# jedeschaud/ct_icp

Measured on NVIDIA B200. Metric: scans/sec (RegisterFrame) on 64-beam ~120k-pt clouds, higher is better.
Workload: dtype f64

## Files before the change

ct_icp_b200/csrc/device_map.cu:

```cuda
#include "device_map.h"

#include <cooperative_groups.h>
#include "gather.cuh"
#include "frame_policy.h"

#include <algorithm>
#include <cstdio>
#include <cstdlib>
#include <numeric>
#include <stdexcept>
#include <vector>

namespace cticp {

#define CT_CUDA_CHECK(expr)                                                                              \
    do {                                                                                                 \
        cudaError_t _e = (expr);                                                                         \
        if (_e != cudaSuccess)                                                                           \
            throw CudaError(std::string(#expr) + ": " + cudaGetErrorString(_e) + " @" + __FILE__ + ":" + \
                            std::to_string(__LINE__));                                                   \
    } while (0)

__global__ void k_clear_level(MapLevel L) {
    const uint32_t cap = L.cap_mask + 1;
// ... 25 lines not shown
                k = atomicCAS(&L.slots[h].key, kEmptyKey, key);
                if (k == kEmptyKey) {
                    atomicAdd(&ctr->num_voxels, 1u);
                    slot = (int) h;
                    break;
                }
            }
            if (k == key) {
                slot = (int) h;
                break;
            }
            h = (h + 1) & L.cap_mask;
        }
        if (slot < 0) {
            atomicExch(&ctr->overflow, 1u);
            next[i] = kNil;
            continue;
        }
        const int old = atomicExch(&L.head[slot], i);
        next[i] = old;
        if (old == kNil) touched[atomicAdd(&ctr->num_touched, 1u)] = (uint32_t) slot;
    }
}
__global__ void k_insert_claim(MapLevel L, MapCounters *ctr, const double *__restrict__ world, const int *d_n,
                               int *__restrict__ next, uint32_t *__restrict__ touched) {
    insert_claim_dev(L, ctr, world, *d_n, next, touched);
}

constexpr int kInsertWarps = 4;
constexpr int kMaxCand = 512;
// ... 45 lines not shown
                    const int v = s_cand[w][a];
                    int rank = 0;
                    for (int b = 0; b < n; ++b) rank += (s_cand[w][b] < v);
                    s_sorted[w][rank] = v;
                }
                m = n;
            } else {
                int best = 0x7fffffff;
                for (int c = L.head[slot]; c != kNil; c = next[c])
                    if (c > last && c < best) best = c;
                if (lane == 0) s_sorted[w][0] = best;
                last = best;
                m = 1;
            }
            __syncwarp();
            for (int a = 0; a < m && count < L.B; ++a) {
                const int c = s_sorted[w][a];
                const double lx = world[3 * c] - ox, ly = world[3 * c + 1] - oy, lz = world[3 * c + 2] - oz;
                bool too_close = false;
                for (int j = lane; j < count; j += 32) {
                    const float4 q = s_pts[w][j];
                    const double dx = (double) q.x - lx, dy = (double) q.y - ly, dz = (double) q.z - lz;
                    const double d2 = dx * dx + dy * dy + dz * dz;
                    too_close |= !(d2 > L.min_dist2);
                }
                const bool reject = __any_sync(0xffffffffu, too_close);
                if (!reject) {
                    if (lane == 0) {
                        const float4 v = make_float4((float) lx, (float) ly, (float) lz, (float) (frame_ordinal + 1));
                        s_pts[w][count] = v;
                        gpts[count] = v;
                    }
                    ++count;
                }
                __syncwarp();
            }
            processed += m;
        }
        if (lane == 0) {
            L.slots[slot].count = (uint32_t) count;
            L.head[slot] = kNil;
            if (count > count0) atomicAdd(&ctr->num_points, (unsigned long long) (count - count0));
        }
        __syncwarp();
        if (L.normals && count > count0 && count >= 5) {
            double sx = 0, sy = 0, sz = 0, sxx = 0, sxy = 0, sxz = 0, syy = 0, syz = 0, szz = 0;
            for (int j = lane; j < count; j += 32) {
                const float4 q = s_pts[w][j];
                const double x = (double) q.x, y = (double) q.y, z = (double) q.z;
                sx += x; sy += y; sz += z;
// ... 66 lines not shown
    const int *d_n;
    double *world;
    Q4 qb, qe;
    V3 tb, te;
    SlerpConsts sc;
    V3 location;
    double max_distance;
    int do_remove, do_insert;
    int *next;
    uint32_t *touched;
    const double *frame_origins;
    int frame_ordinal;
    const FrameVerdict *verdict;
    double *frame_origins_mut;
};
__global__ void __launch_bounds__(kInsertWarps * 32)
k_map_update_fused(FusedUpdateArgs a) {
    namespace cg = cooperative_groups;
    cg::grid_group grid = cg::this_grid();
    __shared__ CommitScratch sc;
    if (a.verdict) {
        const FrameVerdict &v = *a.verdict;
        const int action = v.action;
        if (action != kFrameEvict && action != kFrameInsert) return;
        a.qb = Q4{v.state.qb[0], v.state.qb[1], v.state.qb[2], v.state.qb[3]};
        a.qe = Q4{v.state.qe[0], v.state.qe[1], v.state.qe[2], v.state.qe[3]};
        a.tb = V3{v.state.tb[0], v.state.tb[1], v.state.tb[2]};
        a.te = V3{v.state.te[0], v.state.te[1], v.state.te[2]};
        a.sc = v.sc;
        a.location = a.te;
        a.do_insert = action == kFrameInsert;
// ... 400 lines not shown
```

ct_icp_b200/csrc/engine.cu:

```cuda
#include "engine.h"

#include <algorithm>
#include <atomic>
#include <chrono>
#include <cmath>
#include <cstdio>
#include <cstdlib>
#include <cstring>

#include <emmintrin.h>
#include <xmmintrin.h>

#include <nvtx3/nvToolsExt.h>

namespace cticp {

#define CT_CUDA_CHECK(expr)                                                                              \
    do {                                                                                                 \
        cudaError_t _e = (expr);                                                                         \
        if (_e != cudaSuccess)                                                                           \
            throw CudaError(std::string(#expr) + ": " + cudaGetErrorString(_e) + " @" + __FILE__ + ":" + \
                            std::to_string(__LINE__));                                                   \
    } while (0)

// ... 663 lines not shown
    const bool needs_lo = PackScan(scan, sc.t_min, sc.t_max, pipe_->Staging());
    float4 *stage_lo = needs_lo ? pipe_->StagingLo() : nullptr;
    if (needs_lo) PackLoPlane(scan, sc.t_min, sc.t_max, stage_lo);
    CT_CUDA_CHECK(cudaMalloc(&sc.d_points, sizeof(float4) * n));
    CT_CUDA_CHECK(cudaMemcpyAsync(sc.d_points, pipe_->Staging(), sizeof(float4) * n, cudaMemcpyHostToDevice, stream_));
    if (needs_lo) {
        CT_CUDA_CHECK(cudaMalloc(&sc.d_lo, sizeof(float4) * n));
        CT_CUDA_CHECK(cudaMemcpyAsync(sc.d_lo, stage_lo, sizeof(float4) * n, cudaMemcpyHostToDevice, stream_));
    }
    CT_CUDA_CHECK(cudaStreamSynchronize(stream_));
    staged_.push_back(sc);
    return (int64_t) staged_.size() - 1;
}
void Engine::ClearStaged() {
    CT_CUDA_CHECK(cudaSetDevice(device_));
    CT_CUDA_CHECK(cudaStreamSynchronize(stream_));
    for (auto &sc : staged_) { cudaFree(sc.d_points); cudaFree(sc.d_lo); }
    staged_.clear();
}
void Engine::TimerStart() {
    CT_CUDA_CHECK(cudaSetDevice(device_));
    CT_CUDA_CHECK(cudaEventRecord(timer_ev_[0], stream_));
}
double Engine::TimerStop() {
    CT_CUDA_CHECK(cudaSetDevice(device_));
    CT_CUDA_CHECK(cudaEventRecord(timer_ev_[1], stream_));
    CT_CUDA_CHECK(cudaEventSynchronize(timer_ev_[1]));
    float ms = 0.f;
    CT_CUDA_CHECK(cudaEventElapsedTime(&ms, timer_ev_[0], timer_ev_[1]));
    return (double) ms;
// ... 757 lines not shown
```

ct_icp_b200/csrc/frame_pipeline.cu:

```cuda
#include "frame_pipeline.h"

#include <cooperative_groups.h>
#include <cstdlib>

#include <algorithm>
#include <cstring>

namespace cticp {

#define CT_CUDA_CHECK(expr)                                                                              \
    do {                                                                                                 \
        cudaError_t _e = (expr);                                                                         \
        if (_e != cudaSuccess)                                                                           \
            throw CudaError(std::string(#expr) + ": " + cudaGetErrorString(_e) + " @" + __FILE__ + ":" + \
                            std::to_string(__LINE__));                                                   \
    } while (0)

constexpr unsigned long long kGridEmpty = ~0ull;
constexpr size_t kMaxTiles = 4096;
constexpr int kTileShift = 10, kTile = 1 << kTileShift, kTileThreads = kTile / 4;

__device__ __forceinline__ unsigned long long short_voxel_key(const RawPoint &p, double voxel_size) {
    const double inv = 1.0 / voxel_size;
    const short x = (short) voxel_coord_rcp(p.x, voxel_size, inv);
    const short y = (short) voxel_coord_rcp(p.y, voxel_size, inv);
    const short z = (short) voxel_coord_rcp(p.z, voxel_size, inv);
    return ((unsigned long long) (unsigned short) x << 32) | ((unsigned long long) (unsigned short) y << 16) |
           (unsigned long long) (unsigned short) z;
}

__device__ __forceinline__ void grid_claim_dev(const float4 *pts, const float4 *lo, int n, double voxel_size, int use_perm,
                                               uint64_t seed, uint64_t counter, unsigned long long *keys,
                                               unsigned long long *vals, uint32_t cap_mask, int *__restrict__ slot_of) {
    const Perm perm = perm_make(seed, counter, (uint32_t) max(n, 1));
    for (int i = blockIdx.x * blockDim.x + threadIdx.x; i < n; i += gridDim.x * blockDim.x) {
        const unsigned long long key = short_voxel_key(load_raw(pts, lo, i), voxel_size);
        const uint32_t prio = use_perm ? perm_apply(perm, (uint32_t) i) : (uint32_t) i;
        uint32_t h = hash_key(key) & cap_mask;
        while (true) {
            unsigned long long k = *reinterpret_cast<volatile unsigned long long *>(&keys[h]);
            if (k == kGridEmpty) k = atomicCAS(&keys[h], kGridEmpty, key);
            if (k == kGridEmpty || k == key) break;
            h = (h + 1) & cap_mask;
        }
        atomicMin(&vals[h], ((unsigned long long) prio << 32) | (unsigned) i);
        slot_of[i] = (int) h;
    }
}
__global__ void k_grid_claim(const float4 *__restrict__ pts, const float4 *__restrict__ lo, const int *__restrict__ d_n,
                             double voxel_size, int use_perm, uint64_t seed, uint64_t counter, unsigned long long *keys,
                             unsigned long long *vals, uint32_t cap_mask, int *__restrict__ slot_of) {
    grid_claim_dev(pts, lo, *d_n, voxel_size, use_perm, seed, counter, keys, vals, cap_mask, slot_of);
}
__device__ __forceinline__ void grid_mark_dev(int n, int use_perm, uint64_t seed, uint64_t counter,
                                              const unsigned long long *vals, const int *slot_of, uint32_t *__restrict__ flags,
                                              uint32_t *__restrict__ src, uint32_t *__restrict__ tile_count) {
    const Perm perm = perm_make(seed, counter, (uint32_t) max(n, 1));
    for (int i = blockIdx.x * blockDim.x + threadIdx.x; i < n; i += gridDim.x * blockDim.x) {
        const uint32_t prio = use_perm ? perm_apply(perm, (uint32_t) i) : (uint32_t) i;
        const unsigned long long mine = ((unsigned long long) prio << 32) | (unsigned) i;
        if (vals[slot_of[i]] == mine) {
            flags[prio] = 1u;
            src[prio] = (uint32_t) i;
            atomicAdd(&tile_count[prio >> kTileShift], 1u);
        }
    }
}
__global__ void k_grid_mark(const int *__restrict__ d_n, int use_perm, uint64_t seed, uint64_t counter,
                            const unsigned long long *__restrict__ vals, const int *__restrict__ slot_of,
                            uint32_t *__restrict__ flags, uint32_t *__restrict__ src,
                            uint32_t *__restrict__ tile_count) {
    grid_mark_dev(*d_n, use_perm, seed, counter, vals, slot_of, flags, src, tile_count);
}
struct EmitScratch {
    uint32_t red[2][kTileThreads / 32];
    uint32_t warp[kTileThreads / 32];
    uint32_t before, total;
};
__device__ __forceinline__ uint32_t grid_emit_dev(const float4 *pts, const float4 *lo, const uint32_t *in_src_index, int n,
                                                  const uint32_t *flags, const uint32_t *src, const uint32_t *tile_count,
                                                  int use_perm2, uint64_t seed, uint64_t counter2, int override_alpha,
                                                  float alpha_value, float4 *__restrict__ out, float4 *__restrict__ out_lo,
                                                  uint32_t *__restrict__ out_src_index, int *__restrict__ d_total,
                                                  EmitScratch &sc) {
    uint32_t (&s_red)[2][kTileThreads / 32] = sc.red;
    uint32_t (&s_warp)[kTileThreads / 32] = sc.warp;
    uint32_t &s_before = sc.before, &s_total = sc.total;
    const int num_tiles = (n + kTile - 1) >> kTileShift;
    const int tid = threadIdx.x, lane = tid & 31, w = tid >> 5;
    uint32_t tot = 0;
    for (int t = tid; t < num_tiles; t += kTileThreads) tot += tile_count[t];
#pragma unroll
    for (int o = 16; o > 0; o >>= 1) tot += __shfl_xor_sync(0xffffffffu, tot, o);
    if (lane == 0) s_red[1][w] = tot;
    __syncthreads();
    if (tid == 0) {
        uint32_t b = 0;
        for (int i = 0; i < kTileThreads / 32; ++i) b += s_red[1][i];
        s_total = b;
    }
    __syncthreads();
    const uint32_t total = s_total;
    if (blockIdx.x == 0 && tid == 0) *d_total = (int) total;
    const Perm perm2 = perm_make(seed, counter2, max(total, 1u));

    for (int tile = blockIdx.x; tile < num_tiles; tile += gridDim.x) {
        uint32_t before = 0;
        for (int t = tid; t < tile; t += kTileThreads) before += tile_count[t];
#pragma unroll
        for (int o = 16; o > 0; o >>= 1) before += __shfl_xor_sync(0xffffffffu, before, o);
        __syncthreads();
        if (lane == 0) s_red[0][w] = before;
        const int p0 = (tile << kTileShift) + tid * 4;
        uint32_t v[4];
#pragma unroll
        for (int k = 0; k < 4; ++k) v[k] = (p0 + k < n) ? flags[p0 + k] : 0u;
        const uint32_t tsum = v[0] + v[1] + v[2] + v[3];
        uint32_t incl = tsum;
#pragma unroll
// ... 12 lines not shown
                const uint32_t c = s_warp[i];
                s_warp[i] = run;
                run += c;
            }
        }
        __syncthreads();
        uint32_t excl = s_before + s_warp[w] + (incl - tsum);
#pragma unroll
        for (int k = 0; k < 4; ++k) {
            if (v[k]) {
                const uint32_t dst = (use_perm2 && total > 1) ? perm_apply(perm2, excl) : excl;
                const uint32_t i = src[p0 + k];
                float4 val = pts[i];
                if (override_alpha) val.w = alpha_value;
                out[dst] = val;
                if (out_lo) {
                    float4 l = lo ? lo[i] : make_float4(0.f, 0.f, 0.f, 0.f);
                    if (override_alpha) l.w = 0.f;
                    out_lo[dst] = l;
                }
                out_src_index[dst] = in_src_index ? in_src_index[i] : i;
            }
            excl += v[k];
        }
    }
    return total;
}
__global__ void __launch_bounds__(kTileThreads)
k_grid_emit(const float4 *__restrict__ pts, const float4 *__restrict__ lo, const uint32_t *__restrict__ in_src_index,
            const int *__restrict__ d_n, const uint32_t *__restrict__ flags, const uint32_t *__restrict__ src,
            const uint32_t *__restrict__ tile_count, int use_perm2, uint64_t seed, uint64_t counter2,
            int override_alpha, float alpha_value, float4 *__restrict__ out, float4 *__restrict__ out_lo,
            uint32_t *__restrict__ out_src_index, int *__restrict__ d_total) {
    __shared__ EmitScratch sc;
    grid_emit_dev(pts, lo, in_src_index, *d_n, flags, src, tile_count, use_perm2, seed, counter2, override_alpha, alpha_value,
                  out, out_lo, out_src_index, d_total, sc);
}

struct FusedSampleArgs {
    const float4 *raw;
    const float4 *raw_lo;
    float4 *frame_lo, *kp_lo;
    int *counts;
    double voxel1, voxel2;
    uint64_t seed, c1, c2;
    int override_alpha;
    float alpha_value;
    unsigned long long *grid;
    uint32_t cap1;
    int *slot_of;
    uint32_t *tile1, *flags1, *src1;
    uint32_t *tile2, *flags2, *src2;
    float4 *frame, *keypoints;
    uint32_t *frame_src, *kp_src;
    int pre_cleared;
    uint32_t clear_words;
};
__global__ void __launch_bounds__(kTileThreads)
k_sample_fused(FusedSampleArgs a) {
    namespace cg = cooperative_groups;
    cg::grid_group grid = cg::this_grid();
    __shared__ EmitScratch sc;
    const size_t gtid = (size_t) blockIdx.x * blockDim.x + threadIdx.x, gsize = (size_t) gridDim.x * blockDim.x;
    const int n = a.counts[0];
    if (!a.pre_cleared) {
        for (size_t i = gtid; i < 2 * (size_t) a.cap1; i += gsize) a.grid[i] = kGridEmpty;
        for (size_t i = gtid; i < kMaxTiles + (size_t) n; i += gsize) a.tile1[i] = 0u;
        grid.sync();
    }
    grid_claim_dev(a.raw, a.raw_lo, n, a.voxel1, 1, a.seed, a.c1, a.grid, a.grid + a.cap1, a.cap1 - 1, a.slot_of);
    grid.sync();
    grid_mark_dev(n, 1, a.seed, a.c1, a.grid + a.cap1, a.slot_of, a.flags1, a.src1, a.tile1);
    grid.sync();
    float4 *frame_lo = a.raw_lo ? a.frame_lo : nullptr, *kp_lo = a.raw_lo ? a.kp_lo : nullptr;
    const uint32_t F = grid_emit_dev(a.raw, a.raw_lo, nullptr, n, a.flags1, a.src1, a.tile1, 1, a.seed, a.c2, a.override_alpha,
                                     a.alpha_value, a.frame, frame_lo, a.frame_src, a.counts + 1, sc);
    uint32_t cap2 = 1024;
    while (cap2 < 2 * F) cap2 <<= 1;
    for (size_t i = gtid; i < 2 * (size_t) cap2; i += gsize) a.grid[i] = kGridEmpty;
    for (size_t i = gtid; i < kMaxTiles + (size_t) F; i += gsize) a.tile2[i] = 0u;
    grid.sync();
    grid_claim_dev(a.frame, frame_lo, (int) F, a.voxel2, 0, 0, 0, a.grid, a.grid + cap2, cap2 - 1, a.slot_of);
    grid.sync();
    grid_mark_dev((int) F, 0, 0, 0, a.grid + cap2, a.slot_of, a.flags2, a.src2, a.tile2);
    grid.sync();
    grid_emit_dev(a.frame, frame_lo, a.frame_src, (int) F, a.flags2, a.src2, a.tile2, 0, 0, 0, 0, 0.f, a.keypoints, kp_lo,
                  a.kp_src, a.counts + 2, sc);
    if (a.clear_words) {
        for (size_t i = gtid; i < 2 * (size_t) a.cap1; i += gsize) a.grid[i] = kGridEmpty;
        for (size_t i = gtid; i < (size_t) a.clear_words; i += gsize) a.tile1[i] = 0u;
    }
}
struct AdaptiveBands {
    int num_bands;
    double distance[CTICP_MAX_ADAPTIVE_BANDS];
    double voxel_size[CTICP_MAX_ADAPTIVE_BANDS];
};
__device__ __forceinline__ int adaptive_band(const AdaptiveBands &B, const RawPoint &p, unsigned long long *key_out) {
    const double x = p.x, y = p.y, z = p.z;
    const double dist = sqrt(x * x + y * y + z * z);
    int lw = 0;
    while (lw < B.num_bands && B.distance[lw] < dist) ++lw;
    if (!(dist >= B.distance[0] && dist < B.distance[B.num_bands - 1])) return -1;
    const int band = lw - 1;
// ... 98 lines not shown
}

static uint32_t NextPow2(uint64_t v) {
    uint64_t p = 1;
    while (p < v) p <<= 1;
    return (uint32_t) p;
}

FramePipeline::FramePipeline(size_t max_points, cudaStream_t stream) : stream_(stream), max_points_(max_points) {
    const size_t n = max_points_;
    if (const char *e = getenv("CTICP_SAMPLE_PRECLEAR")) preclear_ = atoi(e) != 0;
    grid_cap_ = std::max<uint32_t>(NextPow2(2 * n), 1024);
    CT_CUDA_CHECK(cudaMallocHost(&h_stage_, sizeof(float4) * n));
    CT_CUDA_CHECK(cudaMallocHost(&h_counts_, sizeof(int) * 8));
    CT_CUDA_CHECK(cudaMalloc(&d_raw_, sizeof(float4) * n));
    CT_CUDA_CHECK(cudaMalloc(&d_frame_, sizeof(float4) * n));
    CT_CUDA_CHECK(cudaMalloc(&d_keypoints_, sizeof(float4) * n));
    CT_CUDA_CHECK(cudaMalloc(&d_tmp_points_, sizeof(float4) * n));
    CT_CUDA_CHECK(cudaMalloc(&d_frame_src_, sizeof(uint32_t) * n));
    CT_CUDA_CHECK(cudaMalloc(&d_kp_src_, sizeof(uint32_t) * n));
    CT_CUDA_CHECK(cudaMalloc(&d_tmp_src_, sizeof(uint32_t) * n));
    CT_CUDA_CHECK(cudaMalloc(&d_grid_, sizeof(unsigned long long) * 2 * (size_t) grid_cap_));
    CT_CUDA_CHECK(cudaMalloc(&d_slot_of_, sizeof(int) * n));
    if ((n + kTile - 1) / kTile > kMaxTiles) throw std::invalid_argument("max_points_per_frame too large");
    CT_CUDA_CHECK(cudaMalloc(&d_tile_count_, sizeof(uint32_t) * (kMaxTiles + n)));
    d_flags_ = d_tile_count_ + kMaxTiles;
    CT_CUDA_CHECK(cudaMalloc(&d_src_, sizeof(uint32_t) * n));
    CT_CUDA_CHECK(cudaMalloc(&d_counts_, sizeof(int) * 8));
    CT_CUDA_CHECK(cudaMalloc(&d_frame_world_, sizeof(double) * 3 * n));
    CT_CUDA_CHECK(cudaMemsetAsync(d_counts_, 0, sizeof(int) * 8, stream_));
    memset(h_counts_, 0, sizeof(int) * 8);
}
FramePipeline::~FramePipeline() {
    cudaFreeHost(h_stage_); cudaFreeHost(h_counts_);
    cudaFree(d_raw_); cudaFree(d_frame_); cudaFree(d_keypoints_); cudaFree(d_tmp_points_);
    cudaFreeHost(h_stage_lo_);
    cudaFree(d_raw_lo_); cudaFree(d_frame_lo_); cudaFree(d_kp_lo_); cudaFree(d_tmp_lo_);
    cudaFree(d_frame_src_); cudaFree(d_kp_src_); cudaFree(d_tmp_src_);
    cudaFree(d_grid_); cudaFree(d_slot_of_); cudaFree(d_tile_count_); cudaFree(d_src_);
    cudaFree(d_counts_); cudaFree(d_frame_world_); cudaFree(d_all_world_); cudaFree(d_adaptive_);
    cudaFree(d_tile2_); cudaFree(d_src2_);
}

int FramePipeline::Blocks(size_t n) const { return (int) std::max<size_t>(1, std::min<size_t>((n + 255) / 256, 148 * 8)); }

void FramePipeline::EnsureLo() {
    if (d_raw_lo_) return;
    CT_CUDA_CHECK(cudaMallocHost(&h_stage_lo_, sizeof(float4) * max_points_));
    CT_CUDA_CHECK(cudaMalloc(&d_raw_lo_, sizeof(float4) * max_points_));
    CT_CUDA_CHECK(cudaMalloc(&d_frame_lo_, sizeof(float4) * max_points_));
    CT_CUDA_CHECK(cudaMalloc(&d_kp_lo_, sizeof(float4) * max_points_));
    CT_CUDA_CHECK(cudaMalloc(&d_tmp_lo_, sizeof(float4) * max_points_));
}

void FramePipeline::UploadLo(size_t n) {
    EnsureLo();
    CT_CUDA_CHECK(cudaMemcpyAsync(d_raw_lo_, h_stage_lo_, sizeof(float4) * n, cudaMemcpyHostToDevice, stream_));
    raw_lo_ = true;
    h2d_bytes_ += sizeof(float4) * n;
}

void FramePipeline::Upload(size_t n) {
    if (n > max_points_) throw CapacityError("scan has more points than max_points_per_frame");
    raw_lo_ = frame_lo_ = distorted_ = false;
    n_ = n;
    h_counts_[0] = (int) n;
    CT_CUDA_CHECK(cudaMemcpyAsync(d_raw_, h_stage_, sizeof(float4) * n, cudaMemcpyHostToDevice, stream_));
    CT_CUDA_CHECK(cudaMemcpyAsync(d_counts_, h_counts_, sizeof(int), cudaMemcpyHostToDevice, stream_));
    h2d_bytes_ = sizeof(float4) * n + sizeof(int);
}

void FramePipeline::UploadBegin(size_t n) {
    if (n > max_points_) throw CapacityError("scan has more points than max_points_per_frame");
    raw_lo_ = frame_lo_ = distorted_ = false;
    n_ = n;
    h_counts_[0] = (int) n;
    CT_CUDA_CHECK(cudaMemcpyAsync(d_counts_, h_counts_, sizeof(int), cudaMemcpyHostToDevice, stream_));
    h2d_bytes_ = sizeof(float4) * n + sizeof(int);
}
void FramePipeline::UploadRange(size_t begin, size_t end) {
    if (end <= begin) return;
    CT_CUDA_CHECK(cudaMemcpyAsync(d_raw_ + begin, h_stage_ + begin, sizeof(float4) * (end - begin), cudaMemcpyHostToDevice, stream_));
}

void FramePipeline::UploadFromDevice(const float4 *d_src, const float4 *d_src_lo, size_t n) {
    if (n > max_points_) throw CapacityError("scan has more points than max_points_per_frame");
    raw_lo_ = frame_lo_ = distorted_ = false;
    n_ = n;
    h_counts_[0] = (int) n;
    CT_CUDA_CHECK(cudaMemcpyAsync(d_raw_, d_src, sizeof(float4) * n, cudaMemcpyDeviceToDevice, stream_));
    if (d_src_lo) {
        EnsureLo();
        CT_CUDA_CHECK(cudaMemcpyAsync(d_raw_lo_, d_src_lo, sizeof(float4) * n, cudaMemcpyDeviceToDevice, stream_));
        raw_lo_ = true;
    }
    CT_CUDA_CHECK(cudaMemcpyAsync(d_counts_, h_counts_, sizeof(int), cudaMemcpyHostToDevice, stream_));
    h2d_bytes_ = sizeof(int);
}

void FramePipeline::GridSelect(const float4 *in, const float4 *in_lo, const uint32_t *in_src, const int *d_n_in,
                               size_t n_upper, double voxel_size, int use_perm1, uint64_t seed, uint64_t c1,
                               int use_perm2, uint64_t c2, int override_alpha, float alpha_value, float4 *out,
                               float4 *out_lo, uint32_t *out_src, int *d_n_out) {
    if (!in_lo) out_lo = nullptr;
    clean_cap_ = 0;
    clean_words_ = 0;
    const uint32_t cap = std::max<uint32_t>(NextPow2(2 * n_upper), 1024);
    unsigned long long *keys = d_grid_, *vals = d_grid_ + cap;
    CT_CUDA_CHECK(cudaMemsetAsync(keys, 0xFF, sizeof(unsigned long long) * 2 * (size_t) cap, stream_));
    const size_t num_tiles = (n_upper + kTile - 1) / kTile;
    CT_CUDA_CHECK(cudaMemsetAsync(d_tile_count_, 0, sizeof(uint32_t) * (kMaxTiles + n_upper), stream_));
    const int blocks = Blocks(n_upper);
// ... 41 lines not shown
    k_grid_emit<<<(int) std::min<size_t>(std::max<size_t>(1, num_tiles), 1184), kTileThreads, 0, stream_>>>(
        in, in_lo, in_src, d_positions, flags, src, tile_count, 0, 0, 0, 0, 0.f, out, out_lo, out_src, d_n_out);
    launches_ += 3;
    if (o.max_num_points > 0) {
        k_clamp_count<<<1, 1, 0, stream_>>>(d_n_out, o.max_num_points + 1);
        launches_ += 1;
    }
    CT_CUDA_CHECK(cudaGetLastError());
}

void FramePipeline::SampleFused(double voxel_size, double sample_voxel_size, uint64_t seed, uint64_t counter1,
                                uint64_t counter2, bool override_alpha, float alpha_value) {
    if (!d_tile2_) {
        CT_CUDA_CHECK(cudaMalloc(&d_tile2_, sizeof(uint32_t) * (kMaxTiles + max_points_)));
        CT_CUDA_CHECK(cudaMalloc(&d_src2_, sizeof(uint32_t) * max_points_));
        int per_sm = 0;
        CT_CUDA_CHECK(cudaOccupancyMaxActiveBlocksPerMultiprocessor(&per_sm, k_sample_fused, kTileThreads, 0));
        int dev = 0, sms = 148;
        cudaGetDevice(&dev);
        cudaDeviceGetAttribute(&sms, cudaDevAttrMultiProcessorCount, dev);
        int want = 4;
        if (const char *e = getenv("CTICP_SAMPLE_CTAS_PER_SM")) want = std::max(1, atoi(e));
        fused_grid_ = std::max(1, std::min(per_sm, want) * sms);
    }
    FusedSampleArgs a;
    a.raw = d_raw_;
    a.raw_lo = d_raw_lo();
    a.frame_lo = d_frame_lo_; a.kp_lo = d_kp_lo_;
    frame_lo_ = raw_lo_;
    a.counts = d_counts_;
    a.voxel1 = voxel_size;
    a.voxel2 = sample_voxel_size;
    a.seed = seed; a.c1 = counter1; a.c2 = counter2;
    a.override_alpha = override_alpha ? 1 : 0;
    a.alpha_value = alpha_value;
    a.grid = d_grid_;
    a.cap1 = std::max<uint32_t>(NextPow2(2 * n_), 1024);
    a.pre_cleared = (preclear_ && clean_cap_ >= a.cap1 && clean_words_ >= kMaxTiles + n_) ? 1 : 0;
    a.clear_words = preclear_ ? (uint32_t) (kMaxTiles + std::min(max_points_, n_ + n_ / 8 + 1024)) : 0u;
    clean_cap_ = preclear_ ? a.cap1 : 0;
    clean_words_ = a.clear_words;
    a.slot_of = d_slot_of_;
    a.tile1 = d_tile_count_; a.flags1 = d_flags_; a.src1 = d_src_;
    a.tile2 = d_tile2_; a.flags2 = d_tile2_ + kMaxTiles; a.src2 = d_src2_;
    a.frame = d_frame_; a.keypoints = d_keypoints_;
    a.frame_src = d_frame_src_; a.kp_src = d_kp_src_;
    void *args[] = {&a};
    CT_CUDA_CHECK(cudaLaunchCooperativeKernel((void *) k_sample_fused, dim3(fused_grid_), dim3(kTileThreads), args, 0, stream_));
    launches_ += 1;
}

void FramePipeline::SubSampleFrame(double voxel_size, uint64_t seed, uint64_t counter1, uint64_t counter2,
                                   bool override_alpha, float alpha_value) {
    GridSelect(d_raw_, d_raw_lo(), nullptr, d_counts_ + 0, n_, voxel_size, 1, seed, counter1, 1, counter2,
               override_alpha ? 1 : 0, alpha_value, d_frame_, d_frame_lo_, d_frame_src_, d_counts_ + 1);
    frame_lo_ = raw_lo_;
}

void FramePipeline::SampleKeypoints(int sampling, double sample_voxel_size, int max_num_keypoints, uint64_t seed,
                                    uint64_t counter, const cticp_adaptive_options *adaptive) {
    if (sampling == CTICP_SAMPLING_ADAPTIVE) {
        if (!adaptive) throw std::invalid_argument("adaptive options missing");
        AdaptiveSelect(*adaptive, d_frame_, d_frame_lo(), d_frame_src_, d_counts_ + 1, n_, d_keypoints_, d_kp_lo_, d_kp_src_,
                       d_counts_ + 2);
    } else if (sampling == CTICP_SAMPLING_GRID) {
        GridSelect(d_frame_, d_frame_lo(), d_frame_src_, d_counts_ + 1, n_, sample_voxel_size, 0, 0, 0, 0, 0, 0, 0.f,
                   d_keypoints_, d_kp_lo_, d_kp_src_, d_counts_ + 2);
    } else {
        k_copy_points<<<Blocks(n_), 256, 0, stream_>>>(d_frame_, d_frame_lo(), d_frame_src_, d_counts_ + 1, d_keypoints_,
// ... 25 lines not shown
    launches_ += 1;
    CT_CUDA_CHECK(cudaGetLastError());
}

void FramePipeline::TransformFrame(const Q4 &qb, const V3 &tb, const Q4 &qe, const V3 &te) {
    k_transform_points<<<Blocks(n_), 256, 0, stream_>>>(d_frame_, d_frame_lo(), d_counts_ + 1, qb, tb, qe, te, slerp_consts(qb, qe), d_frame_world_);
    launches_ += 1;
    CT_CUDA_CHECK(cudaGetLastError());
}

void FramePipeline::EnsureAllWorld() {
    if (!d_all_world_) CT_CUDA_CHECK(cudaMalloc(&d_all_world_, sizeof(double) * 3 * max_points_));
}
void FramePipeline::TransformAll(const Q4 &qb, const V3 &tb, const Q4 &qe, const V3 &te, cudaStream_t stream) {
    EnsureAllWorld();
    k_transform_points<<<Blocks(n_), 256, 0, stream ? stream : stream_>>>(d_raw_, d_raw_lo(), d_counts_ + 0, qb, tb, qe, te, slerp_consts(qb, qe), d_all_world_);
    launches_ += 1;
    CT_CUDA_CHECK(cudaGetLastError());
}

void FramePipeline::TransformInto(const float4 *pts, const float4 *lo, const int *d_n, const Q4 &qb, const V3 &tb,
                                  const Q4 &qe, const V3 &te, double *d_world, cudaStream_t stream) {
    k_transform_points<<<Blocks(n_), 256, 0, stream ? stream : stream_>>>(pts, lo, d_n, qb, tb, qe, te, slerp_consts(qb, qe), d_world);
    launches_ += 1;
    CT_CUDA_CHECK(cudaGetLastError());
}

}
```

ct_icp_b200/csrc/frame_pipeline.h:

```cpp
#pragma once
#include <cuda_runtime.h>

#include <cstdint>

#include "device_map.h"
#include "se3.cuh"

namespace cticp {

class FramePipeline {
public:
    FramePipeline(size_t max_points, cudaStream_t stream);
    ~FramePipeline();
    FramePipeline(const FramePipeline &) = delete;
    FramePipeline &operator=(const FramePipeline &) = delete;

    float4 *Staging() { return h_stage_; }
    void EnsureLo();
    float4 *StagingLo() { EnsureLo(); return h_stage_lo_; }
    const float4 *StagingLoIfAny() const { return raw_lo_ ? h_stage_lo_ : nullptr; }
    void UploadLo(size_t n);
    bool raw_has_lo() const { return raw_lo_; }
    bool frame_has_lo() const { return frame_lo_; }
    bool frame_distorted() const { return distorted_; }
    const float4 *d_raw_lo() const { return raw_lo_ ? d_raw_lo_ : nullptr; }
    const float4 *d_frame_lo() const { return frame_lo_ ? d_frame_lo_ : nullptr; }
    const float4 *d_keypoints_lo() const { return frame_lo_ ? d_kp_lo_ : nullptr; }
    size_t MaxPoints() const { return max_points_; }
    void Upload(size_t n);
    void UploadBegin(size_t n);
    void UploadRange(size_t begin, size_t end);
    void UploadFromDevice(const float4 *d_src, const float4 *d_src_lo, size_t n);

    void SubSampleFrame(double voxel_size, uint64_t seed, uint64_t counter1, uint64_t counter2, bool override_alpha,
                        float alpha_value);
    void SampleFused(double voxel_size, double sample_voxel_size, uint64_t seed, uint64_t counter1, uint64_t counter2,
                     bool override_alpha, float alpha_value);
    void SampleKeypoints(int sampling, double sample_voxel_size, int max_num_keypoints, uint64_t seed, uint64_t counter,
                         const cticp_adaptive_options *adaptive = nullptr);
    void AdaptiveSelect(const cticp_adaptive_options &o, const float4 *in, const float4 *in_lo, const uint32_t *in_src,
                        const int *d_n_in, size_t n_upper, float4 *out, float4 *out_lo, uint32_t *out_src, int *d_n_out);
    void DistortFrame(const Q4 &qb, const V3 &tb, const Q4 &qe, const V3 &te);
    void TransformFrame(const Q4 &qb, const V3 &tb, const Q4 &qe, const V3 &te);
    void TransformAll(const Q4 &qb, const V3 &tb, const Q4 &qe, const V3 &te, cudaStream_t stream = nullptr);
    void TransformInto(const float4 *pts, const float4 *lo, const int *d_n, const Q4 &qb, const V3 &tb, const Q4 &qe,
                       const V3 &te, double *d_world, cudaStream_t stream = nullptr);
    void EnsureAllWorld();

    void QueueCountsReadback();
    const int *h_counts() const { return h_counts_; }
    void SetHostCounts(const int *c) {
        for (int i = 0; i < 4; ++i) h_counts_[i] = c[i];
    }
    const int *d_counts() const { return d_counts_; }

    const float4 *d_raw() const { return d_raw_; }
    const float4 *d_frame() const { return d_frame_; }
    const float4 *d_keypoints() const { return d_keypoints_; }
    float4 *d_keypoints_mut() { return d_keypoints_; }
    const uint32_t *d_frame_src() const { return d_frame_src_; }
    const uint32_t *d_keypoints_src() const { return d_kp_src_; }
    const double *d_frame_world() const { return d_frame_world_; }
    const double *d_all_world() const { return d_all_world_; }
    int *d_count_n() { return d_counts_ + 0; }
    int *d_count_frame() { return d_counts_ + 1; }
    int *d_count_keypoints() { return d_counts_ + 2; }
    size_t n() const { return n_; }
    size_t h2d_bytes() const { return h2d_bytes_; }
    int launches() const { return launches_; }

    void GridSelect(const float4 *in, const float4 *in_lo, const uint32_t *in_src, const int *d_n_in, size_t n_upper,
                    double voxel_size, int use_perm1, uint64_t seed, uint64_t c1, int use_perm2, uint64_t c2,
                    int override_alpha, float alpha_value, float4 *out, float4 *out_lo, uint32_t *out_src, int *d_n_out);
    float4 *d_frame_lo_mut() { EnsureLo(); return d_frame_lo_; }
    float4 *d_raw_mut() { return d_raw_; }
    double *d_frame_world_mut() { return d_frame_world_; }
    float4 *d_frame_mut() { return d_frame_; }
    uint32_t *d_frame_src_mut() { return d_frame_src_; }

private:
    int Blocks(size_t n) const;

    cudaStream_t stream_;
    size_t max_points_, n_ = 0, h2d_bytes_ = 0;
    uint32_t grid_cap_ = 0;
    float4 *h_stage_ = nullptr;
    int *h_counts_ = nullptr;
    float4 *d_raw_ = nullptr, *d_frame_ = nullptr, *d_keypoints_ = nullptr, *d_tmp_points_ = nullptr;
    float4 *h_stage_lo_ = nullptr, *d_raw_lo_ = nullptr, *d_frame_lo_ = nullptr, *d_kp_lo_ = nullptr, *d_tmp_lo_ = nullptr;
    bool raw_lo_ = false, frame_lo_ = false, distorted_ = false;
    uint32_t *d_frame_src_ = nullptr, *d_kp_src_ = nullptr, *d_tmp_src_ = nullptr;
    unsigned long long *d_grid_ = nullptr;
    int *d_slot_of_ = nullptr;
    uint32_t *d_tile_count_ = nullptr, *d_flags_ = nullptr, *d_src_ = nullptr;
    int *d_counts_ = nullptr;
    double *d_frame_world_ = nullptr, *d_all_world_ = nullptr;
    uint32_t *d_tile2_ = nullptr, *d_src2_ = nullptr;
    int fused_grid_ = 0;
    bool preclear_ = true;
    uint32_t clean_cap_ = 0;
    size_t clean_words_ = 0;
    uint32_t *d_adaptive_ = nullptr;
    size_t adaptive_capacity_ = 0;
    int launches_ = 0;
};

}
// ... 1 lines not shown
```

Baseline: 3896.

## Fuse second-level grid claim into emit, warp-dedupe claims, and zero-copy device uploads

Several changes land together. The second voxel-grid claim is folded into the first emit pass using a separate grid2 buffer, which removes a grid sync and a clear pass. Grid claims are deduplicated within a warp via match_any and reduce_min so only one thread per voxel does the atomics. UploadFromDevice now points at the source buffer instead of copying it, with DetachRaw copying it back only when staged buffers are freed. The map commit loads 32 candidates per warp at once and broadcasts them by shuffle, full voxels are skipped at insert time, and the fused update kernel gets a minBlocks launch bound. Risks include extra memory for grid2, possible register spills from the launch bound, and lifetime hazards from aliasing the device source buffer.

```diff
diff --git a/ct_icp_b200/csrc/device_map.cu b/ct_icp_b200/csrc/device_map.cu
--- a/ct_icp_b200/csrc/device_map.cu
+++ b/ct_icp_b200/csrc/device_map.cu
@@ -63,6 +63,10 @@
         }
         if (slot < 0) {
             atomicExch(&ctr->overflow, 1u);
+            next[i] = kNil;
+            continue;
+        }
+        if (L.slots[slot].count >= (uint32_t) L.B) {
             next[i] = kNil;
             continue;
         }
@@ -138,26 +142,34 @@
                 m = 1;
             }
             __syncwarp();
-            for (int a = 0; a < m && count < L.B; ++a) {
-                const int c = s_sorted[w][a];
-                const double lx = world[3 * c] - ox, ly = world[3 * c + 1] - oy, lz = world[3 * c + 2] - oz;
-                bool too_close = false;
-                for (int j = lane; j < count; j += 32) {
-                    const float4 q = s_pts[w][j];
-                    const double dx = (double) q.x - lx, dy = (double) q.y - ly, dz = (double) q.z - lz;
-                    const double d2 = dx * dx + dy * dy + dz * dz;
-                    too_close |= !(d2 > L.min_dist2);
+            for (int a0 = 0; a0 < m && count < L.B; a0 += 32) {
+                double cx = 0.0, cy = 0.0, cz = 0.0;
+                if (a0 + lane < m) {
+                    const int c = s_sorted[w][a0 + lane];
+                    cx = world[3 * c] - ox; cy = world[3 * c + 1] - oy; cz = world[3 * c + 2] - oz;
                 }
-                const bool reject = __any_sync(0xffffffffu, too_close);
-                if (!reject) {
-                    if (lane == 0) {
-                        const float4 v = make_float4((float) lx, (float) ly, (float) lz, (float) (frame_ordinal + 1));
-                        s_pts[w][count] = v;
-                        gpts[count] = v;
+                const int chunk = min(32, m - a0);
+                for (int a = 0; a < chunk && count < L.B; ++a) {
+                    const double lx = __shfl_sync(0xffffffffu, cx, a), ly = __shfl_sync(0xffffffffu, cy, a),
+                                 lz = __shfl_sync(0xffffffffu, cz, a);
+                    bool too_close = false;
+                    for (int j = lane; j < count; j += 32) {
+                        const float4 q = s_pts[w][j];
+                        const double dx = (double) q.x - lx, dy = (double) q.y - ly, dz = (double) q.z - lz;
+                        const double d2 = dx * dx + dy * dy + dz * dz;
+                        too_close |= !(d2 > L.min_dist2);
                     }
-                    ++count;
+                    const bool reject = __any_sync(0xffffffffu, too_close);
+                    if (!reject) {
+                        if (lane == 0) {
+                            const float4 v = make_float4((float) lx, (float) ly, (float) lz, (float) (frame_ordinal + 1));
+                            s_pts[w][count] = v;
+                            gpts[count] = v;
+                        }
+                        ++count;
+                    }
+                    __syncwarp();
                 }
-                __syncwarp();
             }
             processed += m;
         }
@@ -254,7 +266,7 @@
     const FrameVerdict *verdict;
     double *frame_origins_mut;
 };
-__global__ void __launch_bounds__(kInsertWarps * 32)
+__global__ void __launch_bounds__(kInsertWarps * 32, 4)
 k_map_update_fused(FusedUpdateArgs a) {
     namespace cg = cooperative_groups;
     cg::grid_group grid = cg::this_grid();
diff --git a/ct_icp_b200/csrc/engine.cu b/ct_icp_b200/csrc/engine.cu
--- a/ct_icp_b200/csrc/engine.cu
+++ b/ct_icp_b200/csrc/engine.cu
@@ -701,6 +701,7 @@
 }
 void Engine::ClearStaged() {
     CT_CUDA_CHECK(cudaSetDevice(device_));
+    pipe_->DetachRaw();
     CT_CUDA_CHECK(cudaStreamSynchronize(stream_));
     for (auto &sc : staged_) { cudaFree(sc.d_points); cudaFree(sc.d_lo); }
     staged_.clear();
diff --git a/ct_icp_b200/csrc/frame_pipeline.cu b/ct_icp_b200/csrc/frame_pipeline.cu
--- a/ct_icp_b200/csrc/frame_pipeline.cu
+++ b/ct_icp_b200/csrc/frame_pipeline.cu
@@ -29,22 +29,36 @@
            (unsigned long long) (unsigned short) z;
 }
 
+__device__ __forceinline__ uint32_t grid_find_or_insert(unsigned long long *keys, uint32_t cap_mask, unsigned long long key) {
+    uint32_t h = hash_key(key) & cap_mask;
+    while (true) {
+        unsigned long long k = *reinterpret_cast<volatile unsigned long long *>(&keys[h]);
+        if (k == kGridEmpty) k = atomicCAS(&keys[h], kGridEmpty, key);
+        if (k == kGridEmpty || k == key) return h;
+        h = (h + 1) & cap_mask;
+    }
+}
 __device__ __forceinline__ void grid_claim_dev(const float4 *pts, const float4 *lo, int n, double voxel_size, int use_perm,
                                                uint64_t seed, uint64_t counter, unsigned long long *keys,
                                                unsigned long long *vals, uint32_t cap_mask, int *__restrict__ slot_of) {
     const Perm perm = perm_make(seed, counter, (uint32_t) max(n, 1));
-    for (int i = blockIdx.x * blockDim.x + threadIdx.x; i < n; i += gridDim.x * blockDim.x) {
+    const int lane = threadIdx.x & 31;
+    const int warp = (blockIdx.x * blockDim.x + threadIdx.x) >> 5, num_warps = (gridDim.x * blockDim.x) >> 5;
+    for (int base = warp * 32; base < n; base += num_warps * 32) {
+        const int i = base + lane;
+        const unsigned active = __ballot_sync(0xffffffffu, i < n);
+        if (i >= n) continue;
         const unsigned long long key = short_voxel_key(load_raw(pts, lo, i), voxel_size);
         const uint32_t prio = use_perm ? perm_apply(perm, (uint32_t) i) : (uint32_t) i;
-        uint32_t h = hash_key(key) & cap_mask;
-        while (true) {
-            unsigned long long k = *reinterpret_cast<volatile unsigned long long *>(&keys[h]);
-            if (k == kGridEmpty) k = atomicCAS(&keys[h], kGridEmpty, key);
-            if (k == kGridEmpty || k == key) break;
-            h = (h + 1) & cap_mask;
-        }
-        atomicMin(&vals[h], ((unsigned long long) prio << 32) | (unsigned) i);
-        slot_of[i] = (int) h;
+        const unsigned peers = __match_any_sync(active, key);
+        const uint32_t best = __reduce_min_sync(peers, prio);
+        const bool leader = prio == best;
+        uint32_t h = 0;
+        if (leader) {
+            h = grid_find_or_insert(keys, cap_mask, key);
+            atomicMin(&vals[h], ((unsigned long long) prio << 32) | (unsigned) i);
+        }
+        slot_of[i] = leader ? (int) h : -1;
     }
 }
 __global__ void k_grid_claim(const float4 *__restrict__ pts, const float4 *__restrict__ lo, const int *__restrict__ d_n,
@@ -57,9 +71,11 @@
                                               uint32_t *__restrict__ src, uint32_t *__restrict__ tile_count) {
     const Perm perm = perm_make(seed, counter, (uint32_t) max(n, 1));
     for (int i = blockIdx.x * blockDim.x + threadIdx.x; i < n; i += gridDim.x * blockDim.x) {
+        const int slot = slot_of[i];
+        if (slot < 0) continue;
         const uint32_t prio = use_perm ? perm_apply(perm, (uint32_t) i) : (uint32_t) i;
         const unsigned long long mine = ((unsigned long long) prio << 32) | (unsigned) i;
-        if (vals[slot_of[i]] == mine) {
+        if (vals[slot] == mine) {
             flags[prio] = 1u;
             src[prio] = (uint32_t) i;
             atomicAdd(&tile_count[prio >> kTileShift], 1u);
@@ -76,13 +92,24 @@
     uint32_t red[2][kTileThreads / 32];
     uint32_t warp[kTileThreads / 32];
     uint32_t before, total;
+};
+__device__ __forceinline__ uint32_t grid_cap_for(uint32_t n) {
+    uint32_t cap = 1024;
+    while (cap < 2 * n) cap <<= 1;
+    return cap;
+}
+struct NextClaim {
+    double voxel_size;
+    unsigned long long *grid;
+    int *slot_of;
+    uint32_t *tile;
 };
 __device__ __forceinline__ uint32_t grid_emit_dev(const float4 *pts, const float4 *lo, const uint32_t *in_src_index, int n,
                                                   const uint32_t *flags, const uint32_t *src, const uint32_t *tile_count,
                                                   int use_perm2, uint64_t seed, uint64_t counter2, int override_alpha,
                                                   float alpha_value, float4 *__restrict__ out, float4 *__restrict__ out_lo,
                                                   uint32_t *__restrict__ out_src_index, int *__restrict__ d_total,
-                                                  EmitScratch &sc) {
+                                                  EmitScratch &sc, const NextClaim *next = nullptr) {
     uint32_t (&s_red)[2][kTileThreads / 32] = sc.red;
     uint32_t (&s_warp)[kTileThreads / 32] = sc.warp;
     uint32_t &s_before = sc.before, &s_total = sc.total;
@@ -103,6 +130,12 @@
     const uint32_t total = s_total;
     if (blockIdx.x == 0 && tid == 0) *d_total = (int) total;
     const Perm perm2 = perm_make(seed, counter2, max(total, 1u));
+    uint32_t next_mask = 0;
+    if (next) {
+        next_mask = grid_cap_for(total) - 1;
+        const size_t words = kMaxTiles + (size_t) total;
+        for (size_t t = (size_t) blockIdx.x * blockDim.x + tid; t < words; t += (size_t) gridDim.x * blockDim.x) next->tile[t] = 0u;
+    }
 
     for (int tile = blockIdx.x; tile < num_tiles; tile += gridDim.x) {
         uint32_t before = 0;
@@ -145,12 +178,19 @@
                 float4 val = pts[i];
                 if (override_alpha) val.w = alpha_value;
                 out[dst] = val;
+                RawPoint r{f32_to_f64(val.x), f32_to_f64(val.y), f32_to_f64(val.z), 0.0};
                 if (out_lo) {
                     float4 l = lo ? lo[i] : make_float4(0.f, 0.f, 0.f, 0.f);
                     if (override_alpha) l.w = 0.f;
                     out_lo[dst] = l;
+                    r.x += (double) l.x; r.y += (double) l.y; r.z += (double) l.z;
                 }
                 out_src_index[dst] = in_src_index ? in_src_index[i] : i;
+                if (next) {
+                    const uint32_t h = grid_find_or_insert(next->grid, next_mask, short_voxel_key(r, next->voxel_size));
+                    atomicMin(&next->grid[next_mask + 1 + h], ((unsigned long long) dst << 32) | dst);
+                    next->slot_of[dst] = (int) h;
+                }
             }
             excl += v[k];
         }
@@ -172,12 +212,14 @@
     const float4 *raw;
     const float4 *raw_lo;
     float4 *frame_lo, *kp_lo;
+    int n;
     int *counts;
     double voxel1, voxel2;
     uint64_t seed, c1, c2;
     int override_alpha;
     float alpha_value;
     unsigned long long *grid;
+    unsigned long long *grid2;
     uint32_t cap1;
     int *slot_of;
     uint32_t *tile1, *flags1, *src1;
@@ -193,9 +235,11 @@
     cg::grid_group grid = cg::this_grid();
     __shared__ EmitScratch sc;
     const size_t gtid = (size_t) blockIdx.x * blockDim.x + threadIdx.x, gsize = (size_t) gridDim.x * blockDim.x;
-    const int n = a.counts[0];
+    const int n = a.n;
+    if (blockIdx.x == 0 && threadIdx.x == 0) a.counts[0] = n;
     if (!a.pre_cleared) {
         for (size_t i = gtid; i < 2 * (size_t) a.cap1; i += gsize) a.grid[i] = kGridEmpty;
+        for (size_t i = gtid; i < 2 * (size_t) a.cap1; i += gsize) a.grid2[i] = kGridEmpty;
         for (size_t i = gtid; i < kMaxTiles + (size_t) n; i += gsize) a.tile1[i] = 0u;
         grid.sync();
     }
@@ -204,21 +248,18 @@
     grid_mark_dev(n, 1, a.seed, a.c1, a.grid + a.cap1, a.slot_of, a.flags1, a.src1, a.tile1);
     grid.sync();
     float4 *frame_lo = a.raw_lo ? a.frame_lo : nullptr, *kp_lo = a.raw_lo ? a.kp_lo : nullptr;
+    const NextClaim claim2{a.voxel2, a.grid2, a.slot_of, a.tile2};
     const uint32_t F = grid_emit_dev(a.raw, a.raw_lo, nullptr, n, a.flags1, a.src1, a.tile1, 1, a.seed, a.c2, a.override_alpha,
-                                     a.alpha_value, a.frame, frame_lo, a.frame_src, a.counts + 1, sc);
-    uint32_t cap2 = 1024;
-    while (cap2 < 2 * F) cap2 <<= 1;
-    for (size_t i = gtid; i < 2 * (size_t) cap2; i += gsize) a.grid[i] = kGridEmpty;
-    for (size_t i = gtid; i < kMaxTiles + (size_t) F; i += gsize) a.tile2[i] = 0u;
+                                     a.alpha_value, a.frame, frame_lo, a.frame_src, a.counts + 1, sc, &claim2);
+    const uint32_t cap2 = grid_cap_for(F);
     grid.sync();
-    grid_claim_dev(a.frame, frame_lo, (int) F, a.voxel2, 0, 0, 0, a.grid, a.grid + cap2, cap2 - 1, a.slot_of);
-    grid.sync();
-    grid_mark_dev((int) F, 0, 0, 0, a.grid + cap2, a.slot_of, a.flags2, a.src2, a.tile2);
+    grid_mark_dev((int) F, 0, 0, 0, a.grid2 + cap2, a.slot_of, a.flags2, a.src2, a.tile2);
     grid.sync();
     grid_emit_dev(a.frame, frame_lo, a.frame_src, (int) F, a.flags2, a.src2, a.tile2, 0, 0, 0, 0, 0.f, a.keypoints, kp_lo,
                   a.kp_src, a.counts + 2, sc);
     if (a.clear_words) {
         for (size_t i = gtid; i < 2 * (size_t) a.cap1; i += gsize) a.grid[i] = kGridEmpty;
+        for (size_t i = gtid; i < 2 * (size_t) cap2; i += gsize) a.grid2[i] = kGridEmpty;
         for (size_t i = gtid; i < (size_t) a.clear_words; i += gsize) a.tile1[i] = 0u;
     }
 }
@@ -347,6 +388,7 @@
     CT_CUDA_CHECK(cudaMallocHost(&h_stage_, sizeof(float4) * n));
     CT_CUDA_CHECK(cudaMallocHost(&h_counts_, sizeof(int) * 8));
     CT_CUDA_CHECK(cudaMalloc(&d_raw_, sizeof(float4) * n));
+    raw_ = d_raw_;
     CT_CUDA_CHECK(cudaMalloc(&d_frame_, sizeof(float4) * n));
     CT_CUDA_CHECK(cudaMalloc(&d_keypoints_, sizeof(float4) * n));
     CT_CUDA_CHECK(cudaMalloc(&d_tmp_points_, sizeof(float4) * n));
@@ -372,7 +414,7 @@
     cudaFree(d_frame_src_); cudaFree(d_kp_src_); cudaFree(d_tmp_src_);
     cudaFree(d_grid_); cudaFree(d_slot_of_); cudaFree(d_tile_count_); cudaFree(d_src_);
     cudaFree(d_counts_); cudaFree(d_frame_world_); cudaFree(d_all_world_); cudaFree(d_adaptive_);
-    cudaFree(d_tile2_); cudaFree(d_src2_);
+    cudaFree(d_tile2_); cudaFree(d_src2_); cudaFree(d_grid2_);
 }
 
 int FramePipeline::Blocks(size_t n) const { return (int) std::max<size_t>(1, std::min<size_t>((n + 255) / 256, 148 * 8)); }
@@ -390,12 +432,14 @@
     EnsureLo();
     CT_CUDA_CHECK(cudaMemcpyAsync(d_raw_lo_, h_stage_lo_, sizeof(float4) * n, cudaMemcpyHostToDevice, stream_));
     raw_lo_ = true;
+    raw_lo_view_ = d_raw_lo_;
     h2d_bytes_ += sizeof(float4) * n;
 }
 
 void FramePipeline::Upload(size_t n) {
     if (n > max_points_) throw CapacityError("scan has more points than max_points_per_frame");
-    raw_lo_ = frame_lo_ = distorted_ = false;
+    raw_lo_ = frame_lo_ = distorted_ = count_n_pending_ = false;
+    raw_ = d_raw_;
     n_ = n;
     h_counts_[0] = (int) n;
     CT_CUDA_CHECK(cudaMemcpyAsync(d_raw_, h_stage_, sizeof(float4) * n, cudaMemcpyHostToDevice, stream_));
@@ -405,7 +449,8 @@
 
 void FramePipeline::UploadBegin(size_t n) {
     if (n > max_points_) throw CapacityError("scan has more points than max_points_per_frame");
-    raw_lo_ = frame_lo_ = distorted_ = false;
+    raw_lo_ = frame_lo_ = distorted_ = count_n_pending_ = false;
+    raw_ = d_raw_;
     n_ = n;
     h_counts_[0] = (int) n;
     CT_CUDA_CHECK(cudaMemcpyAsync(d_counts_, h_counts_, sizeof(int), cudaMemcpyHostToDevice, stream_));
@@ -418,17 +463,32 @@
 
 void FramePipeline::UploadFromDevice(const float4 *d_src, const float4 *d_src_lo, size_t n) {
     if (n > max_points_) throw CapacityError("scan has more points than max_points_per_frame");
-    raw_lo_ = frame_lo_ = distorted_ = false;
+    frame_lo_ = distorted_ = false;
     n_ = n;
-    h_counts_[0] = (int) n;
-    CT_CUDA_CHECK(cudaMemcpyAsync(d_raw_, d_src, sizeof(float4) * n, cudaMemcpyDeviceToDevice, stream_));
-    if (d_src_lo) {
+    raw_ = d_src;
+    raw_lo_view_ = d_src_lo;
+    raw_lo_ = d_src_lo != nullptr;
+    count_n_pending_ = true;
+    h2d_bytes_ = 0;
+}
+
+void FramePipeline::DetachRaw() {
+    if (raw_ == d_raw_) return;
+    CT_CUDA_CHECK(cudaMemcpyAsync(d_raw_, raw_, sizeof(float4) * n_, cudaMemcpyDeviceToDevice, stream_));
+    if (raw_lo_) {
         EnsureLo();
-        CT_CUDA_CHECK(cudaMemcpyAsync(d_raw_lo_, d_src_lo, sizeof(float4) * n, cudaMemcpyDeviceToDevice, stream_));
-        raw_lo_ = true;
-    }
+        CT_CUDA_CHECK(cudaMemcpyAsync(d_raw_lo_, raw_lo_view_, sizeof(float4) * n_, cudaMemcpyDeviceToDevice, stream_));
+    }
+    raw_ = d_raw_;
+    raw_lo_view_ = d_raw_lo_;
+}
+
+void FramePipeline::EnsureCountN() {
+    if (!count_n_pending_) return;
+    h_counts_[0] = (int) n_;
     CT_CUDA_CHECK(cudaMemcpyAsync(d_counts_, h_counts_, sizeof(int), cudaMemcpyHostToDevice, stream_));
-    h2d_bytes_ = sizeof(int);
+    h2d_bytes_ += sizeof(int);
+    count_n_pending_ = false;
 }
 
 void FramePipeline::GridSelect(const float4 *in, const float4 *in_lo, const uint32_t *in_src, const int *d_n_in,
@@ -500,6 +560,8 @@
     if (!d_tile2_) {
         CT_CUDA_CHECK(cudaMalloc(&d_tile2_, sizeof(uint32_t) * (kMaxTiles + max_points_)));
         CT_CUDA_CHECK(cudaMalloc(&d_src2_, sizeof(uint32_t) * max_points_));
+        CT_CUDA_CHECK(cudaMalloc(&d_grid2_, sizeof(unsigned long long) * 2 * (size_t) grid_cap_));
+        CT_CUDA_CHECK(cudaMemsetAsync(d_grid2_, 0xFF, sizeof(unsigned long long) * 2 * (size_t) grid_cap_, stream_));
         int per_sm = 0;
         CT_CUDA_CHECK(cudaOccupancyMaxActiveBlocksPerMultiprocessor(&per_sm, k_sample_fused, kTileThreads, 0));
         int dev = 0, sms = 148;
@@ -510,8 +572,10 @@
         fused_grid_ = std::max(1, std::min(per_sm, want) * sms);
     }
     FusedSampleArgs a;
-    a.raw = d_raw_;
+    a.raw = raw_;
     a.raw_lo = d_raw_lo();
+    a.n = (int) n_;
+    count_n_pending_ = false;
     a.frame_lo = d_frame_lo_; a.kp_lo = d_kp_lo_;
     frame_lo_ = raw_lo_;
     a.counts = d_counts_;
@@ -521,6 +585,7 @@
     a.override_alpha = override_alpha ? 1 : 0;
     a.alpha_value = alpha_value;
     a.grid = d_grid_;
+    a.grid2 = d_grid2_;
     a.cap1 = std::max<uint32_t>(NextPow2(2 * n_), 1024);
     a.pre_cleared = (preclear_ && clean_cap_ >= a.cap1 && clean_words_ >= kMaxTiles + n_) ? 1 : 0;
     a.clear_words = preclear_ ? (uint32_t) (kMaxTiles + std::min(max_points_, n_ + n_ / 8 + 1024)) : 0u;
@@ -538,7 +603,8 @@
 
 void FramePipeline::SubSampleFrame(double voxel_size, uint64_t seed, uint64_t counter1, uint64_t counter2,
                                    bool override_alpha, float alpha_value) {
-    GridSelect(d_raw_, d_raw_lo(), nullptr, d_counts_ + 0, n_, voxel_size, 1, seed, counter1, 1, counter2,
+    EnsureCountN();
+    GridSelect(raw_, d_raw_lo(), nullptr, d_counts_ + 0, n_, voxel_size, 1, seed, counter1, 1, counter2,
                override_alpha ? 1 : 0, alpha_value, d_frame_, d_frame_lo_, d_frame_src_, d_counts_ + 1);
     frame_lo_ = raw_lo_;
 }
@@ -594,7 +660,7 @@
 }
 void FramePipeline::TransformAll(const Q4 &qb, const V3 &tb, const Q4 &qe, const V3 &te, cudaStream_t stream) {
     EnsureAllWorld();
-    k_transform_points<<<Blocks(n_), 256, 0, stream ? stream : stream_>>>(d_raw_, d_raw_lo(), d_counts_ + 0, qb, tb, qe, te, slerp_consts(qb, qe), d_all_world_);
+    k_transform_points<<<Blocks(n_), 256, 0, stream ? stream : stream_>>>(raw_, d_raw_lo(), d_counts_ + 0, qb, tb, qe, te, slerp_consts(qb, qe), d_all_world_);
     launches_ += 1;
     CT_CUDA_CHECK(cudaGetLastError());
 }
diff --git a/ct_icp_b200/csrc/frame_pipeline.h b/ct_icp_b200/csrc/frame_pipeline.h
--- a/ct_icp_b200/csrc/frame_pipeline.h
+++ b/ct_icp_b200/csrc/frame_pipeline.h
@@ -23,7 +23,7 @@
     bool raw_has_lo() const { return raw_lo_; }
     bool frame_has_lo() const { return frame_lo_; }
     bool frame_distorted() const { return distorted_; }
-    const float4 *d_raw_lo() const { return raw_lo_ ? d_raw_lo_ : nullptr; }
+    const float4 *d_raw_lo() const { return raw_lo_ ? raw_lo_view_ : nullptr; }
     const float4 *d_frame_lo() const { return frame_lo_ ? d_frame_lo_ : nullptr; }
     const float4 *d_keypoints_lo() const { return frame_lo_ ? d_kp_lo_ : nullptr; }
     size_t MaxPoints() const { return max_points_; }
@@ -31,6 +31,7 @@
     void UploadBegin(size_t n);
     void UploadRange(size_t begin, size_t end);
     void UploadFromDevice(const float4 *d_src, const float4 *d_src_lo, size_t n);
+    void DetachRaw();
 
     void SubSampleFrame(double voxel_size, uint64_t seed, uint64_t counter1, uint64_t counter2, bool override_alpha,
                         float alpha_value);
@@ -54,7 +55,7 @@
     }
     const int *d_counts() const { return d_counts_; }
 
-    const float4 *d_raw() const { return d_raw_; }
+    const float4 *d_raw() const { return raw_; }
     const float4 *d_frame() const { return d_frame_; }
     const float4 *d_keypoints() const { return d_keypoints_; }
     float4 *d_keypoints_mut() { return d_keypoints_; }
@@ -73,13 +74,13 @@
                     double voxel_size, int use_perm1, uint64_t seed, uint64_t c1, int use_perm2, uint64_t c2,
                     int override_alpha, float alpha_value, float4 *out, float4 *out_lo, uint32_t *out_src, int *d_n_out);
     float4 *d_frame_lo_mut() { EnsureLo(); return d_frame_lo_; }
-    float4 *d_raw_mut() { return d_raw_; }
     double *d_frame_world_mut() { return d_frame_world_; }
     float4 *d_frame_mut() { return d_frame_; }
     uint32_t *d_frame_src_mut() { return d_frame_src_; }
 
 private:
     int Blocks(size_t n) const;
+    void EnsureCountN();
 
     cudaStream_t stream_;
     size_t max_points_, n_ = 0, h2d_bytes_ = 0;
@@ -89,8 +90,10 @@
     float4 *d_raw_ = nullptr, *d_frame_ = nullptr, *d_keypoints_ = nullptr, *d_tmp_points_ = nullptr;
     float4 *h_stage_lo_ = nullptr, *d_raw_lo_ = nullptr, *d_frame_lo_ = nullptr, *d_kp_lo_ = nullptr, *d_tmp_lo_ = nullptr;
     bool raw_lo_ = false, frame_lo_ = false, distorted_ = false;
+    const float4 *raw_ = nullptr, *raw_lo_view_ = nullptr;
+    bool count_n_pending_ = false;
     uint32_t *d_frame_src_ = nullptr, *d_kp_src_ = nullptr, *d_tmp_src_ = nullptr;
-    unsigned long long *d_grid_ = nullptr;
+    unsigned long long *d_grid_ = nullptr, *d_grid2_ = nullptr;
     int *d_slot_of_ = nullptr;
     uint32_t *d_tile_count_ = nullptr, *d_flags_ = nullptr, *d_src_ = nullptr;
     int *d_counts_ = nullptr;
```

Measured after the change: 4179, median of 6. +7.3%, better.
